# dlwns147/amq

Measured on AMD Instinct MI355X. Metric: decode tokens/s, Llama-2-7B AMQ mixed 2/3/4-bit avg-3-bit, batch 1, higher is better.
Workload: dtype f16; 1 GPU; Llama-2-7B shapes, synthesized avg-3.0-bit per-layer arch (bits_usage 2.982), batch 1 decode after a 64-token prefill, one stream per GPU; parallelism=replicas x1, prompt=64, group_size=128

## Files before the change

amq_amd/csrc/amq_decode.hip:

```cpp
#include <type_traits>
#include "amq_common.cuh"
#include "amq_kernels.h"

namespace amq {

__device__ __forceinline__ float wave_sum_f(float v) {
#pragma unroll
    for (int off = 32; off > 0; off >>= 1) v += __shfl_xor(v, off);
    return v;
}
__device__ __forceinline__ float wave_max_f(float v) {
#pragma unroll
    for (int off = 32; off > 0; off >>= 1) v = fmaxf(v, __shfl_xor(v, off));
    return v;
}

template <bool FRAG>
__global__ __launch_bounds__(256) void rmsnorm_kernel(const _Float16* x, const _Float16* gamma, _Float16* y, int M, int K, float eps) {
    __shared__ float red[4];
    const int m = blockIdx.x;
    const bool live = m < M;
    const _Float16* xr = x + (size_t)(live ? m : 0) * K;
    float ss = 0.f;
    for (int c = threadIdx.x; c < (K >> 3); c += 256) {
// ... 75 lines not shown
                *(h8*)(xlm + 8 * c) = r;
            }
        }
    }
    __syncthreads();
    const int gw = blockIdx.x * WV + wave, nw = gridDim.x * WV;
    const int steps = (K + 511) >> 9;
    for (int row = gw; row < N; row += nw) {
        const _Float16* wr = W + (size_t)row * K + 8 * lane;
        float acc[M];
#pragma unroll
        for (int m = 0; m < M; ++m) acc[m] = 0.f;
        for (int s = 0; s < steps; s += 4) {
            u4 buf[4];
#pragma unroll
            for (int j = 0; j < 4; ++j)
                if (s + j < steps && (s + j) * 512 + 8 * lane < K) buf[j] = AMQ_STREAM_LOAD((const u4*)(wr + (size_t)(s + j) * 512));
#pragma unroll
            for (int j = 0; j < 4; ++j) {
                if (s + j < steps && (s + j) * 512 + 8 * lane < K) {
                    const uint32_t wv[4] = {buf[j].x, buf[j].y, buf[j].z, buf[j].w};
#pragma unroll
                    for (int m = 0; m < M; ++m) {
                        const h8 xv = *(const h8*)(xl + (size_t)m * K + (s + j) * 512 + 8 * lane);
#pragma unroll
                        for (int p = 0; p < 4; ++p) {
                            h2 xp = {xv[2 * p], xv[2 * p + 1]};
                            acc[m] = __builtin_amdgcn_fdot2(as_h2(wv[p]), xp, acc[m], false);
                        }
                    }
                }
            }
        }
#pragma unroll
        for (int m = 0; m < M; ++m) {
            const float t = wave_sum_f(acc[m]);
            if (lane == 0) {
                _Float16 o = (_Float16)t;
                if (bias) o = o + bias[row];
                y[(size_t)m * N + row] = o;
            }
        }
    }
}

template <bool NORM, int M>
static hipError_t launch_gemv_f16w_m(const void* x, const void* W, const void* bias, void* y, const void* gamma, float eps,
                                     int N, int K, hipStream_t st) {
    const size_t lds = (size_t)M * K * 2 + 64;
    constexpr int WV = M == 1 ? F16W_WAVES : 16;
    auto k = gemv_f16w_kernel<NORM, M, WV>;
    if (lds > 64 * 1024) {
        hipError_t e = hipFuncSetAttribute((const void*)k, hipFuncAttributeMaxDynamicSharedMemorySize, (int)lds);
        if (e != hipSuccess) return e;
    }
    hipLaunchKernelGGL(k, dim3(M == 1 ? 1024 : 512), dim3(WV * 64), lds, st, (const _Float16*)x, (const _Float16*)W, (const _Float16*)bias,
                       (_Float16*)y, (const _Float16*)gamma, eps, N, K);
    return hipGetLastError();
}

template <bool NORM>
static hipError_t launch_gemv_f16w_n(const void* x, const void* W, const void* bias, void* y, const void* gamma, float eps,
                                     int M, int N, int K, hipStream_t st) {
    switch (M) {
        case 1: return launch_gemv_f16w_m<NORM, 1>(x, W, bias, y, gamma, eps, N, K, st);
        case 2: return launch_gemv_f16w_m<NORM, 2>(x, W, bias, y, gamma, eps, N, K, st);
        case 3: return launch_gemv_f16w_m<NORM, 3>(x, W, bias, y, gamma, eps, N, K, st);
        case 4: return launch_gemv_f16w_m<NORM, 4>(x, W, bias, y, gamma, eps, N, K, st);
        case 5: return launch_gemv_f16w_m<NORM, 5>(x, W, bias, y, gamma, eps, N, K, st);
        case 6: return launch_gemv_f16w_m<NORM, 6>(x, W, bias, y, gamma, eps, N, K, st);
        case 7: return launch_gemv_f16w_m<NORM, 7>(x, W, bias, y, gamma, eps, N, K, st);
        default: return launch_gemv_f16w_m<NORM, 8>(x, W, bias, y, gamma, eps, N, K, st);
    }
}

hipError_t launch_gemv_f16w(const void* x, const void* W, const void* bias, void* y, const void* gamma, float eps,
                            int N, int K, hipStream_t st, int M) {
    StreamDevice sd_(st);
    if (gamma) return launch_gemv_f16w_n<true>(x, W, bias, y, gamma, eps, M, N, K, st);
    return launch_gemv_f16w_n<false>(x, W, bias, y, nullptr, eps, M, N, K, st);
}

constexpr int TAIL_MAX_SUPPRESS = 8;
template <bool SEQ>
__global__ __launch_bounds__(1024) void decode_tail_kernel(const _Float16* logits, int vocab, const _Float16* embed, int hidden,
                                                            long long* token, int* pos, _Float16* x, const _Float16* rope_table,
                                                            _Float16* rope_cur, int rope_rows, const int* suppress) {
    __shared__ float smax[16];
    __shared__ int sidx[16];
    __shared__ int stok, spos;
    const int tid = threadIdx.x;
    logits += (size_t)blockIdx.x * vocab;
    token += blockIdx.x;
    x += (size_t)blockIdx.x * hidden;
    if (SEQ) {
        pos = (int*)((char*)pos + (size_t)blockIdx.x * STEP_STRIDE);
        if (rope_cur) rope_cur = (_Float16*)((char*)rope_cur + (size_t)blockIdx.x * STEP_STRIDE);
    } else if (blockIdx.x != 0) rope_cur = nullptr;
    float best = -INFINITY;
    int bi = 0x7fffffff;
    int sup[TAIL_MAX_SUPPRESS];
#pragma unroll
    for (int j = 0; j < TAIL_MAX_SUPPRESS; ++j) sup[j] = suppress ? suppress[j] : -1;
    auto allowed = [&](int idx) {
        bool ok = true;
#pragma unroll
        for (int j = 0; j < TAIL_MAX_SUPPRESS; ++j) ok = ok && idx != sup[j];
        return ok;
    };
    const int chunks = vocab >> 3;
    for (int c = tid; c < chunks; c += 1024) {
        const h8 v = *(const h8*)(logits + 8 * c);
#pragma unroll
        for (int e = 0; e < 8; ++e) {
            const float f = (float)v[e];
            if (f > best && (!suppress || allowed(8 * c + e))) { best = f; bi = 8 * c + e; }
        }
    }
    for (int i = 8 * chunks + tid; i < vocab; i += 1024) {
        const float f = (float)logits[i];
        if ((f > best || (f == best && i < bi)) && (!suppress || allowed(i))) { best = f; bi = i; }
    }
#pragma unroll
    for (int off = 32; off > 0; off >>= 1) {
        const float ob = __shfl_xor(best, off);
        const int oi = __shfl_xor(bi, off);
        if (ob > best || (ob == best && oi < bi)) { best = ob; bi = oi; }
    }
    if ((tid & 63) == 0) { smax[tid >> 6] = best; sidx[tid >> 6] = bi; }
    __syncthreads();
    if (tid == 0) {
        float b = smax[0];
        int ix = sidx[0];
        for (int w = 1; w < 16; ++w)
            if (smax[w] > b || (smax[w] == b && sidx[w] < ix)) { b = smax[w]; ix = sidx[w]; }
        if (ix == 0x7fffffff) ix = 0;
        stok = ix;
        token[0] = (long long)ix;
        if (SEQ || blockIdx.x == 0) {
            spos = pos[0] + 1;
            if (rope_table && spos > rope_rows) spos = rope_rows;
            pos[0] = spos;
        }
    }
    __syncthreads();
    if (rope_cur && tid < 128) {
        const int rr = spos < rope_rows ? spos : rope_rows - 1;
        rope_cur[tid] = rope_table[(size_t)rr * 128 + tid];
    }
    const _Float16* row = embed + (size_t)stok * hidden;
    for (int c = tid; c < (hidden >> 3); c += 1024) *(h8*)(x + 8 * c) = *(const h8*)(row + 8 * c);
}

hipError_t launch_decode_tail(const void* logits, int vocab, const void* embed, int hidden, void* token, void* pos, void* x,
                              const void* rope_table, void* rope_cur, int rope_rows, hipStream_t st, int batch, const void* suppress, bool seq) {
    hipLaunchKernelGGL(seq ? decode_tail_kernel<true> : decode_tail_kernel<false>, dim3(batch), dim3(1024), 0, st, (const _Float16*)logits, vocab,
                       (const _Float16*)embed, hidden, (long long*)token, (int*)pos, (_Float16*)x, (const _Float16*)rope_table, (_Float16*)rope_cur,
                       rope_rows, (const int*)suppress);
    return hipGetLastError();
}

template <bool SEQ>
__global__ __launch_bounds__(256) void set_token_kernel(const long long* token_in, int n_in, const _Float16* embed, int vocab, int hidden, long long* token,
                                                         const int* pos, _Float16* x, const _Float16* rope_table, _Float16* rope_cur, int rope_rows) {
    const int b = blockIdx.x, tid = threadIdx.x;
    long long t = token_in[n_in == 1 ? 0 : b];
    t = t < 0 ? 0 : t >= vocab ? vocab - 1 : t;
    if (tid == 0) token[b] = t;
    if (SEQ) {
        pos = (const int*)((const char*)pos + (size_t)b * STEP_STRIDE);
        if (rope_cur) rope_cur = (_Float16*)((char*)rope_cur + (size_t)b * STEP_STRIDE);
    }
    if ((SEQ || b == 0) && rope_cur && tid < 128) {
        int p = pos[0];
        p = p < 0 ? 0 : p < rope_rows ? p : rope_rows - 1;
        rope_cur[tid] = rope_table[(size_t)p * 128 + tid];
    }
    const _Float16* row = embed + (size_t)t * hidden;
    _Float16* xr = x + (size_t)b * hidden;
    for (int c = tid; c < (hidden >> 3); c += 256) *(h8*)(xr + 8 * c) = *(const h8*)(row + 8 * c);
}

hipError_t launch_set_token(const void* token_in, int n_in, const void* embed, int vocab, int hidden, void* token, const void* pos, void* x,
                            const void* rope_table, void* rope_cur, int rope_rows, int batch, hipStream_t st, bool seq) {
    hipLaunchKernelGGL(seq ? set_token_kernel<true> : set_token_kernel<false>, dim3(batch), dim3(256), 0, st, (const long long*)token_in, n_in,
                       (const _Float16*)embed, vocab, hidden, (long long*)token, (const int*)pos, (_Float16*)x, (const _Float16*)rope_table,
                       (_Float16*)rope_cur, rope_rows);
    return hipGetLastError();
}

constexpr int ATT_D = 128;

__device__ __forceinline__ void rope_cs(float theta, int pos, int i, _Float16* c16, _Float16* s16) {
    const float inv_freq = 1.0f / powf(theta, (float)(2 * i) / (float)ATT_D);
    float sn, cs;
    sincosf((float)pos * inv_freq, &sn, &cs);
    *c16 = (_Float16)cs;
    *s16 = (_Float16)sn;
}


constexpr int ATT_THREADS = 512;
constexpr int ATT_GROUPS = ATT_THREADS / 16;
constexpr int ATT_PF = 12;
#ifndef AMQ_ATT_SPEC
#define AMQ_ATT_SPEC 2
#endif
constexpr int ATT_SPEC = AMQ_ATT_SPEC;

struct AttnRest {
    void* out; const void* rope_table; int pos; float rope_theta;
#ifdef AMQ_STAMP
    unsigned long long* stamps;
#endif
};
struct AttnRestQkn : AttnRest { QkNorm nrm; };
template <bool QKN> using AttnRestT = std::conditional_t<QKN, AttnRestQkn, AttnRest>;
#ifdef AMQ_STAMP
extern unsigned long long* g_stamp_ptr;
#define ATT_STAMP(slot_) do { if (rest.stamps && threadIdx.x == 0) rest.stamps[(size_t)blockIdx.x * 16 + (slot_)] = __builtin_amdgcn_s_memrealtime(); } while (0)
#else
#define ATT_STAMP(slot_) do { } while (0)
#endif

constexpr int ATT_ROWS_MAX = 8;
constexpr int ATT_ROWS_LDS = 2 * (ATT_ROWS_MAX - 1) * ATT_D * 2;
template <bool SEQ, bool ROWS = false, bool QKN = false>
__global__ __launch_bounds__(ATT_THREADS) void attn_decode_kernel(void* p_kc, void* p_vc, const void* p_state, int p_heads,
                                                                   int p_max_seq, const void* p_q, const void* p_k,
                                                                   const void* p_v, AttnRestT<QKN> rest) {
    const void* const p_state0 = p_state;
    if (SEQ) p_state = (const char*)p_state + (size_t)blockIdx.y * STEP_STRIDE;
    extern __shared__ __attribute__((aligned(16))) unsigned char smem[];
    _Float16* qs = (_Float16*)smem;
    _Float16* ks = (_Float16*)smem + ATT_D;
    _Float16* vs = (_Float16*)smem + 2 * ATT_D;
    float* sc = (float*)(smem + 6 * ATT_D);
    __shared__ float red[2 * ATT_THREADS / 64];
    __shared__ float part[ATT_GROUPS][ATT_D];
// ... 137 lines not shown
        if (ATT_GROUPS * i < T) {
            const int t = grp + ATT_GROUPS * i;
            float sv;
            if constexpr (ROWS) {
                h8 kv = krow[i];
                if (t == pos) kv = knew;
                else if (t >= p0 && t < pos) kv = *(const h8*)(kd + (t - p0) * ATT_D + 8 * l16);
                sv = score(kv);
            } else sv = score(t == pos ? knew : krow[i]);
            if (t < T && l16 == 0) sc[t] = sv;
        }
    }
    for (int t = grp + ATT_GROUPS * ATT_PF; t < T; t += ATT_GROUPS) {
        h8 kv;
        if constexpr (ROWS) kv = (t == pos) ? knew : t >= p0 ? *(const h8*)(kd + (t - p0) * ATT_D + 8 * l16) : *(const h8*)(kc + (size_t)t * ATT_D + 8 * l16);
        else kv = (t == pos) ? knew : *(const h8*)(kc + (size_t)t * ATT_D + 8 * l16);
        const float sv = score(kv);
        if (l16 == 0) sc[t] = sv;
    }
    __syncthreads();
    ATT_STAMP(3);
    float lmax = -INFINITY;
    for (int t = tid; t < T; t += ATT_THREADS) lmax = fmaxf(lmax, sc[t]);
    lmax = wave_max_dpp(lmax);
    if ((tid & 63) == 0) red[tid >> 6] = lmax;
    __syncthreads();
    float gmax = red[0];
#pragma unroll
    for (int w = 1; w < ATT_THREADS / 64; ++w) gmax = fmaxf(gmax, red[w]);
    float lsum = 0.f;
    for (int t = tid; t < T; t += ATT_THREADS) {
        const float e = __expf(sc[t] - gmax);
        sc[t] = e;
        lsum += e;
    }
    lsum = wave_sum_dpp(lsum);
    if ((tid & 63) == 0) red[ATT_THREADS / 64 + (tid >> 6)] = lsum;
    __syncthreads();
    float tot = 0.f;
#pragma unroll
    for (int w = 0; w < ATT_THREADS / 64; ++w) tot += red[ATT_THREADS / 64 + w];
    const float inv = 1.0f / tot;
    ATT_STAMP(4);

    float o[8] = {0, 0, 0, 0, 0, 0, 0, 0};
    const h8 vnew = *(const h8*)(vs + 8 * l16);
#pragma unroll
    for (int i = 0; i < ATT_PF; ++i) {
        const int t = grp + ATT_GROUPS * i;
        if (ATT_GROUPS * i < T && t < T) {
            const _Float16 p16 = (_Float16)(sc[t] * inv);
            h8 vv;
            if constexpr (ROWS) {
                vv = vrow[i];
                if (t == pos) vv = vnew;
                else if (t >= p0 && t < pos) vv = *(const h8*)(vd + (t - p0) * ATT_D + 8 * l16);
            } else vv = (t == pos) ? vnew : vrow[i];
#pragma unroll
            for (int e = 0; e < 8; ++e) o[e] += (float)p16 * (float)vv[e];
        }
    }
    for (int t = grp + ATT_GROUPS * ATT_PF; t < T; t += ATT_GROUPS) {
        const _Float16 p16 = (_Float16)(sc[t] * inv);
        h8 vv;
        if constexpr (ROWS) vv = (t == pos) ? vnew : t >= p0 ? *(const h8*)(vd + (t - p0) * ATT_D + 8 * l16) : *(const h8*)(vc + (size_t)t * ATT_D + 8 * l16);
        else vv = (t == pos) ? vnew : *(const h8*)(vc + (size_t)t * ATT_D + 8 * l16);
#pragma unroll
        for (int e = 0; e < 8; ++e) o[e] += (float)p16 * (float)vv[e];
    }
#pragma unroll
    for (int e = 0; e < 8; ++e) part[grp][8 * l16 + e] = o[e];
    __syncthreads();
    ATT_STAMP(5);
    if (tid < ATT_D) {
        float acc = 0.f;
#pragma unroll
        for (int g = 0; g < ATT_GROUPS; ++g) acc += part[g][tid];
        _Float16* out = (_Float16*)rest.out + ((size_t)b * n_heads + h) * ATT_D;
        out[tid] = (_Float16)acc;
    }
    ATT_STAMP(6);
}

struct AttnSplit { float* ws; int* tickets; int n_splits; };
constexpr int ATT_WS_STRIDE = ATT_D + 4;

#ifndef AMQ_ATT_NT
#define AMQ_ATT_NT 1
#endif
#if AMQ_ATT_NT
#define ATT_KV_LOAD(p) __builtin_nontemporal_load((const h8*)(p))
#else
#define ATT_KV_LOAD(p) (*(const h8*)(p))
#endif
template <int RING, bool SEQ, bool ROWS = false, bool QKN = false>
__global__ __launch_bounds__(ATT_THREADS) void attn_decode_split_kernel(void* p_kc, void* p_vc, const void* p_state, int p_heads,
                                                                         int p_max_seq, const void* p_q, const void* p_k,
                                                                         const void* p_v, AttnRestT<QKN> rest, AttnSplit sp) {
    const void* const p_state0 = p_state;
    if (SEQ) p_state = (const char*)p_state + (size_t)blockIdx.y * STEP_STRIDE;
    extern __shared__ __attribute__((aligned(16))) unsigned char smem[];
    _Float16* qs = (_Float16*)smem;
    _Float16* ks = (_Float16*)smem + ATT_D;
    _Float16* vs = (_Float16*)smem + 2 * ATT_D;
    float* sc = (float*)(smem + 6 * ATT_D);
    __shared__ float red[2 * ATT_THREADS / 64];
    __shared__ float part[ATT_GROUPS][ATT_D];
    __shared__ int last_flag;
    const int b = blockIdx.y, z = blockIdx.z, tid = threadIdx.x;
    const int cb = ROWS ? 0 : b;
    const int n_heads = p_heads & 0xFF, n_kv_heads = (p_heads >> 8) & 0xFF, max_seq = p_max_seq;
    int h = blockIdx.x;
    if (n_kv_heads != n_heads && (n_kv_heads & 7) == 0) {
        const int G = n_heads / n_kv_heads, x = h & 7, j = h >> 3;
        h = (x + 8 * (j / G)) * G + j % G;
    }
    const bool cur_mode = (p_heads >> 16) & 1;
    const void* p_cur = cur_mode ? p_state : nullptr;
    int pos;
    if (cur_mode) pos = *(const int*)((const char*)p_state + 256);
    else if (p_state) pos = *(const int*)p_state;
    else pos = rest.pos;
    const int group = n_heads / n_kv_heads;
    const int kvh = h / group;
    const int grp = tid >> 4, l16 = tid & 15;
    const _Float16* q = (const _Float16*)p_q + ((size_t)b * n_heads + h) * ATT_D;
    const _Float16* kn = (const _Float16*)p_k + ((size_t)b * n_kv_heads + kvh) * ATT_D;
    const _Float16* vn = (const _Float16*)p_v + ((size_t)b * n_kv_heads + kvh) * ATT_D;
    _Float16* kc = (_Float16*)p_kc + ((size_t)cb * n_kv_heads + kvh) * (size_t)max_seq * ATT_D;
    _Float16* vc = (_Float16*)p_vc + ((size_t)cb * n_kv_heads + kvh) * (size_t)max_seq * ATT_D;

    _Float16 q0 = 0, q1 = 0, k0 = 0, k1 = 0, v0 = 0, v1 = 0;
    h2 cs_cur = {(_Float16)1.f, (_Float16)0.f}, cs_tab = {(_Float16)1.f, (_Float16)0.f};
    _Float16 gq0 = 0, gq1 = 0, gk0 = 0, gk1 = 0;
    if (tid < 64) {
        q0 = q[tid]; q1 = q[tid + 64];
        k0 = kn[tid]; k1 = kn[tid + 64];
        if (p_cur) cs_cur = ((const h2*)p_cur)[tid];
        v0 = vn[tid]; v1 = vn[tid + 64];
        if constexpr (QKN) {
            const _Float16* const gq = (const _Float16*)rest.nrm.q_gamma;
            const _Float16* const gk = (const _Float16*)rest.nrm.k_gamma;
            gq0 = gq[tid]; gq1 = gq[tid + 64];
            gk0 = gk[tid]; gk1 = gk[tid + 64];
        }
    }
    const int p0 = ROWS ? pos - b : pos;
    if (pos < 0 || pos >= max_seq || (ROWS && p0 < 0)) {
        if (cur_mode && tid == 0 && z == 0) *(int*)((char*)const_cast<void*>(p_state) + 260) = 1;
        return;
    }
    const int T = pos + 1;
    int chunk = (((T + sp.n_splits - 1) / sp.n_splits) + 31) & ~31;
    chunk = chunk < ATT_MIN_CHUNK ? ATT_MIN_CHUNK : chunk;
    const int n_act = (T + chunk - 1) / chunk;
    if (z >= n_act) return;
    const int t0 = z * chunk;
    const int t1 = t0 + chunk < T ? t0 + chunk : T;
    const int Tl = t1 - t0;
    const bool has_new = t1 == T;
    if (tid < 64 && !p_cur && rest.rope_table) cs_tab = ((const h2*)rest.rope_table)[(size_t)pos * 64 + tid];
    const int last_old = ROWS ? (p0 > 0 ? p0 - 1 : 0) : (pos > 0 ? pos - 1 : 0);
    int chunk_max = (((max_seq + sp.n_splits - 1) / sp.n_splits) + 31) & ~31;
    chunk_max = chunk_max < ATT_MIN_CHUNK ? ATT_MIN_CHUNK : chunk_max;
    _Float16* const kd = (_Float16*)(smem + 6 * ATT_D + (size_t)chunk_max * 4);
    _Float16* const vd = kd + (ATT_ROWS_MAX - 1) * ATT_D;
// ... 406 lines not shown
    for (int e = 0; e < 8; ++e) {
        const float gf = (float)gv[e];
        const _Float16 sg = (_Float16)(gf / (1.0f + __expf(-gf)));
        r[e] = sg * uv[e];
    }
    o[idx] = r;
}

hipError_t launch_silu_mul(const void* gate, const void* up, void* out, long n, hipStream_t st) {
    const long n8 = n >> 3;
    hipLaunchKernelGGL(silu_mul_kernel, dim3((unsigned)((n8 + 255) / 256)), dim3(256), 0, st, (const h8*)gate, (const h8*)up,
                       (h8*)out, n8);
    return hipGetLastError();
}

static int att_chunk_max(int max_seq, int n_splits) {
    int c = (((max_seq + n_splits - 1) / n_splits) + 31) & ~31;
    return c < ATT_MIN_CHUNK ? ATT_MIN_CHUNK : c;
}

template <bool QKN>
static AttnRestT<QKN> attn_rest(const AttnArgs& a, void* stamps) {
    AttnRestT<QKN> rest{};
    rest.out = a.out; rest.rope_table = a.rope_table; rest.pos = a.pos; rest.rope_theta = a.rope_theta;
#ifdef AMQ_STAMP
    rest.stamps = (unsigned long long*)stamps;
#endif
    (void)stamps;
    if constexpr (QKN) rest.nrm = a.norm;
    return rest;
}

template <int RING, bool QKN = false>
static hipError_t launch_attn_decode_split_ring(const AttnArgs& a, int batch, int n_splits, void* ws, void* tickets, size_t lds, hipStream_t st) {
    const auto kern = a.rows ? attn_decode_split_kernel<RING, true, true, QKN> : a.seq ? attn_decode_split_kernel<RING, true, false, QKN> : attn_decode_split_kernel<RING, false, false, QKN>;
    if (a.rows) lds += ATT_ROWS_LDS;
    if (lds > 64 * 1024) {
        hipError_t e = hipFuncSetAttribute((const void*)kern, hipFuncAttributeMaxDynamicSharedMemorySize, (int)lds);
        if (e != hipSuccess) return e;
    }
    const AttnRestT<QKN> rest = attn_rest<QKN>(a, nullptr);
    AttnSplit sp{(float*)ws, (int*)tickets, n_splits};
    const bool cur = a.rope_cur != nullptr;
    hipLaunchKernelGGL(kern, dim3(a.n_heads, batch, n_splits), dim3(ATT_THREADS), lds, st, a.kcache, a.vcache,
                       cur ? a.rope_cur : (const void*)a.pos_dev, a.n_heads | (a.n_kv_heads << 8) | ((int)cur << 16), a.max_seq,
                       a.q, a.k, a.v, rest, sp);
    return hipGetLastError();
}

hipError_t launch_attn_decode_split(const AttnArgs& a, int batch, int n_splits, void* ws, void* tickets, hipStream_t st) {
    if (!a.rows && attn_decode_takes_gqa(a.n_heads, a.n_kv_heads, a.max_seq, n_splits)) return launch_attn_decode_gqa(a, batch, n_splits, ws, tickets, st);
    StreamDevice sd_(st);
    const size_t lds = 6 * ATT_D + (size_t)att_chunk_max(a.max_seq, n_splits) * 4;
#ifndef AMQ_ATT_RING_WIDE
#define AMQ_ATT_RING_WIDE 12
#endif
#ifndef AMQ_ATT_RING_NARROW
#define AMQ_ATT_RING_NARROW 4
#endif
    const bool wide = (long)a.n_heads * batch * n_splits <= 256;
    if (a.norm.q_gamma) {
        if (wide) return launch_attn_decode_split_ring<AMQ_ATT_RING_WIDE, true>(a, batch, n_splits, ws, tickets, lds, st);
        return launch_attn_decode_split_ring<AMQ_ATT_RING_NARROW, true>(a, batch, n_splits, ws, tickets, lds, st);
    }
    if (wide) return launch_attn_decode_split_ring<AMQ_ATT_RING_WIDE>(a, batch, n_splits, ws, tickets, lds, st);
    return launch_attn_decode_split_ring<AMQ_ATT_RING_NARROW>(a, batch, n_splits, ws, tickets, lds, st);
}

template <bool QKN>
static hipError_t launch_attn_decode_t(const AttnArgs& a, int batch, hipStream_t st) {
    StreamDevice sd_(st);
    const size_t lds = a.rows ? ((6 * ATT_D + (size_t)a.max_seq * 4 + 15) & ~(size_t)15) + ATT_ROWS_LDS : 6 * ATT_D + (size_t)a.max_seq * 4;
    const auto kern = a.rows ? attn_decode_kernel<true, true, QKN> : a.seq ? attn_decode_kernel<true, false, QKN> : attn_decode_kernel<false, false, QKN>;
    if (lds > 64 * 1024) {
        hipError_t e = hipFuncSetAttribute((const void*)kern, hipFuncAttributeMaxDynamicSharedMemorySize, (int)lds);
        if (e != hipSuccess) return e;
    }
#ifdef AMQ_STAMP
    const AttnRestT<QKN> rest = attn_rest<QKN>(a, g_stamp_ptr);
#else
    const AttnRestT<QKN> rest = attn_rest<QKN>(a, nullptr);
#endif
    const bool cur = a.rope_cur != nullptr;
    hipLaunchKernelGGL(kern, dim3(a.n_heads, batch), dim3(ATT_THREADS), lds, st, a.kcache, a.vcache,
                       cur ? a.rope_cur : (const void*)a.pos_dev, a.n_heads | (a.n_kv_heads << 8) | ((int)cur << 16), a.max_seq,
                       a.q, a.k, a.v, rest);
    return hipGetLastError();
}

hipError_t launch_attn_decode(const AttnArgs& a, int batch, hipStream_t st) {
    return a.norm.q_gamma ? launch_attn_decode_t<true>(a, batch, st) : launch_attn_decode_t<false>(a, batch, st);
}

}
```

amq_amd/llama.py:

```python
import math
from typing import NamedTuple

import torch

from . import ops
from .arch import MODEL_CONFIGS, arch_bits, rope_inv_freq, uniform_arch
from .hqq_format import HQQWeights

EPS = 1e-5
ROPE_THETA = 10000.0


class _Lin:
    __slots__ = ("qn", "mn", "bits", "mode", "N", "K", "bias", "perm", "out_ids", "W_out", "Kp")

    def __init__(self, qn, mn, bits, mode, N, K, bias=None, perm=None, out_ids=None, W_out=None, Kp=None):
        self.qn, self.mn, self.bits, self.mode, self.N, self.K, self.bias = qn, mn, bits, mode, N, K, bias
        self.perm, self.out_ids, self.W_out, self.Kp = perm, out_ids, W_out, K if Kp is None else Kp

    @property
    def owq(self):
        return self.W_out is not None

    def seg(self, y, residual=None, act=False):
# ... 44 lines not shown
            g = torch.cuda.CUDAGraph()
            keep = torch.zeros(1, device=dev)
            with torch.cuda.graph(g, stream=side, capture_error_mode="thread_local"):
                keep += 1
        side.synchronize()
    _GRAPH_STATE_PRIMED.add(key)


def capture_graph(dev, fn, restore=None):
    side = torch.cuda.Stream(device=dev)
    side.wait_stream(torch.cuda.current_stream(dev))
    with torch.cuda.stream(side):
        fn()
        side.synchronize()
        if restore is not None:
            restore()
        g = torch.cuda.CUDAGraph()
        with _no_gc(), torch.cuda.graph(g, stream=side, capture_error_mode="thread_local"):
            fn()
    torch.cuda.current_stream(dev).wait_stream(side)
    return g


def _ints(values, n, lo, hi, message):
    each = [int(values)] * n if isinstance(values, int) else [int(v) for v in (values.reshape(-1).tolist() if isinstance(values, torch.Tensor) else values)]
    if len(each) != n or not all(lo <= v <= hi for v in each):
        raise ValueError(message.format(got=each))
    return each


NORM_FUSED, NORM_LAUNCH, NORM_FROM_SUMS = "fused", "launch", "sums"
DOWN_FUSED, DOWN_GEMV, DOWN_GEMV_SUMS, DOWN_GEMM = "silu_mul prologue", "silu_mul + gemv", "silu_mul + gemv leaving sums", "silu_mul + gemm"


class StepPlan(NamedTuple):
    first_norm: str
    norm: str
    down: str
    staged: bool = False

    @property
    def block_norm(self):
        return self.first_norm if self.norm == NORM_FROM_SUMS and self.down != DOWN_GEMV_SUMS else self.norm


def step_plan(R, H, I, fine, rows_h, rows_i, rows_i_phased, norm_sums=True, norm_fused_rows=4, down_fused_rows=1, rows_q=None):
    own = NORM_LAUNCH if R > norm_fused_rows else NORM_FUSED
    sums = norm_sums and 2 <= R <= 8 and not fine and 2048 <= H <= 8192 and I >= 2048 and R <= rows_h and (rows_q is None or R <= rows_q)
    if R <= min(rows_i, down_fused_rows):
        down = DOWN_FUSED
    elif R <= rows_i_phased:
        down = DOWN_GEMV_SUMS if sums else DOWN_GEMV
    else:
        down = DOWN_GEMM
    return StepPlan(own, NORM_FROM_SUMS if sums else own, down)


class _held_back:

    def __init__(self, runner, ids, hold):
        self.runner, self.ids, self.held = runner, tuple(ids), bool(hold)

    def __enter__(self):
        self.before = self.runner.suppressed
        if self.held:
            self.runner.set_suppressed(self.before + tuple(e for e in self.ids if e not in self.before))
        return self

    def release(self):
        if self.held:
            self.runner.set_suppressed(self.before)
            self.held = False

    def __exit__(self, *exc):
        self.runner.set_suppressed(self.before)
        return False


class QuantLlama:
    ENGINE_MAX_SEQ = 512
    DOWN_FUSED_ROWS = 1
    NORM_FUSED_ROWS = 4
    GATE_ACT = True
    NORM_SUMS = True
    FUSE_QKV_ATTN = False
    ROWS_GQA_FROM = 2048
    kv_bits = 16
    ENGINE_DEFAULT = False
    all_logits = False
    fine = False
    owq = False

    @classmethod
    def rows_attention_grouped(cls, n_heads, n_kv_heads, max_seq):
        if cls.ROWS_GQA_FROM is None or n_kv_heads < 1 or n_heads % n_kv_heads:
            return False
        return 2 <= n_heads // n_kv_heads <= 16 and max_seq >= cls.ROWS_GQA_FROM

    def __init__(self, config, arch_linear=None, device="cuda:0", max_seq=256, seed=0, synthetic=True,
                 hqq_layers=None, dense=None, batch=1, engine=None, prebuilt=None, group=128, rope=None, ragged=False, lookup=0, ngram_max=2,
                 lookup_sampling=False, kv_bits=16):
        if isinstance(config, str):
            config = MODEL_CONFIGS[config]
        if kv_bits not in (8, 16):
            raise ValueError(f"kv_bits must be 16 (fp16 cache) or 8 (int8 rows with a scale per row), got {kv_bits!r}")
        self.kv_bits = int(kv_bits)
        if self.kv_bits == 8:
            if ragged:
                raise ValueError("kv_bits=8: the 8-bit attention kernel keeps one position for the batch: not offered with ragged=True")
            if lookup:
                raise ValueError("kv_bits=8: a verify step runs 2 .. 8 rows of one sequence, the 8-bit attention kernel one: not offered with lookup=")
            if config.get("qk_norm"):
                raise ValueError("kv_bits=8: the 8-bit attention kernel has no per-head q / k norm: not offered for a qk_norm model")
            if engine:
                raise ValueError("kv_bits=8: the decode engine reads an fp16 cache")
            if self.FUSE_QKV_ATTN:
                raise ValueError("kv_bits=8: the fused q/k/v + attention launch reads an fp16 cache")
        if not 1 <= int(batch) <= 8:
            raise ValueError("batch must be 1..8")
        self.B = int(batch)
        self.ragged = bool(ragged)
        self.lookup = int(lookup or 0)
        self.lookup_sampling = bool(lookup_sampling)
        if self.lookup_sampling and not self.lookup:
            raise ValueError("lookup_sampling: sampled verify steps need a runner built with lookup=D (a plain runner samples after set_sampling)")
        if self.lookup:
            if not 1 <= self.lookup <= ops.LOOKUP_MAX_ROWS - 1:
                raise ValueError(f"lookup: 1..{ops.LOOKUP_MAX_ROWS - 1} drafts per step (the 2 .. 8-row launches), got {lookup}")
            if not 1 <= int(ngram_max) <= 4:
                raise ValueError(f"ngram_max must be 1..4, got {ngram_max}")
            if self.B != 1:
                raise ValueError("lookup: the rows of a step are the drafts of ONE sequence (batch 1); batches are not served")
            if self.ragged:
                raise ValueError("lookup: a ragged runner's step-state blocks are sequences, a lookup runner's are the rows of one sequence: not offered with ragged=True")
            if engine:
                raise ValueError("lookup: the decode engine runs one row per launch; a verify step runs 2 .. 8")
            if self.FUSE_QKV_ATTN:
                raise ValueError("lookup: the fused q/k/v + attention launch runs one row; a verify step runs 2 .. 8")
        self.ngram_max = int(ngram_max)
        self.R = self.lookup + 1 if self.lookup else self.B
        if self.ragged and engine:
            raise ValueError("the decode engine keeps one position (batch 1): not offered with ragged=True")
        if self.ragged and self.FUSE_QKV_ATTN:
            raise ValueError("the fused q/k/v + attention launch keeps one position (batch 1): not offered with ragged=True")
        self.cfg = config
        self.dev = torch.device(device)
        _prime_graph_state(self.dev)
        self.H = config["hidden_size"]
        self.I = config["intermediate_size"]
        self.nh, self.nkv = config["num_heads"], config["num_kv_heads"]
        if config["head_dim"] != 128:
            raise ValueError("head_dim must be 128")
        self.kvd = self.nkv * 128
        self.qd = self.nh * 128
        self.qk_norm = bool(config.get("qk_norm"))
        self.nb = config["n_block"]
        self.vocab = config["vocab_size"]
        self.max_seq = max_seq
        self.eps = float(config.get("rms_norm_eps", EPS))
        self.theta = float(config.get("rope_theta", ROPE_THETA))
        arch_linear = arch_linear or uniform_arch(config, 4)["linear"]
        self.arch_linear = arch_linear
        gen = torch.Generator(device=self.dev).manual_seed(seed)
        dev = self.dev

        def lin(block, name):
# ... 184 lines not shown
            if "RMSNorm" not in type(m).__name__ or w is None or tuple(w.shape) != (128,):
                raise ValueError(f"{where}.{name}: expected an RMSNorm over the 128 values of a head, got {type(m).__name__}"
                                 f"{'' if w is None else ' of width ' + 'x'.join(str(d) for d in w.shape)}")
            m_eps = getattr(m, "variance_epsilon", getattr(m, "eps", None))
            if m_eps is None or float(m_eps) != eps:
                raise ValueError(f"{where}.{name}: eps {m_eps} is not the model's rms_norm_eps {eps} (the runner keeps one eps)")

    @classmethod
    def from_hf(cls, model, max_seq=256, batch=1, engine=None, ragged=False, lookup=0, ngram_max=2, lookup_sampling=False, kv_bits=16):
        from .quant_linear import HIPOWQLinear, HIPQuantLinear
        cfg, rope = cls.check_hf(model, max_seq)
        layers = model.model.layers
        pre, arch_linear = {}, {name: [] for name in cfg["linear"]}
        dev = None
        f16 = lambda t: t.detach() if t.dtype is torch.float16 else t.detach().to(torch.float16)
        for b, layer in enumerate(layers):
            for name in cfg["linear"]:
                parent, attr = name.split(".")
                m = getattr(getattr(layer, parent), attr)
                if isinstance(m, HIPOWQLinear) and m.inner.qweight.is_cuda:
                    i = m.inner
                    if i.is_bf16:
                        raise ValueError(f"model.layers.{b}.{name}: a bfloat16 module -- the decode runner is fp16")
                    if m.perm.dtype is not torch.int32 or m.out_ids.dtype is not torch.int32 or m.W_out.dtype is not torch.float16 or \
                            tuple(m.W_out.shape) != (m.outfeatures, m.n_out) or m.perm.numel() != i.infeatures or m.out_ids.numel() != m.n_out:
                        raise ValueError(f"model.layers.{b}.{name}: the OWQ layer's perm / out_ids / W_out do not have the shapes of its packed layer")
                    dev = dev or i.qweight.device
                    pre[(b, name)] = _Lin(i.qweight, i.meta, i.bits, i.mode, m.outfeatures, m.infeatures, None if i.bias is None else f16(i.bias),
                                          perm=m.perm.contiguous(), out_ids=m.out_ids.contiguous(), W_out=m.W_out.contiguous(), Kp=i.infeatures)
                    arch_linear[name].append(i.bits)
                    continue
                if not isinstance(m, HIPQuantLinear) or not m.qweight.is_cuda:
                    raise ValueError(f"model.layers.{b}.{name}: expected a HIPQuantLinear on the GPU (run prepare_for_inference first)")
                if m.is_bf16:
                    raise ValueError(f"model.layers.{b}.{name}: a bfloat16 module -- the decode runner is fp16 (the reference's kernels are, ft.py:62); "
                                     "bf16 models run through the modules' own forward")
                dev = dev or m.qweight.device
                pre[(b, name)] = _Lin(m.qweight, m.meta, m.bits, m.mode, m.outfeatures, m.infeatures, None if m.bias is None else f16(m.bias))
                arch_linear[name].append(m.bits)
        dense = {"embed": f16(model.model.embed_tokens.weight), "lm_head": f16(model.lm_head.weight), "norm": f16(model.model.norm.weight),
                 "ln1": [f16(l.input_layernorm.weight) for l in layers], "ln2": [f16(l.post_attention_layernorm.weight) for l in layers]}
        if cfg.get("qk_norm"):
            dense["qn"] = [f16(l.self_attn.q_norm.weight).contiguous() for l in layers]
            dense["kn"] = [f16(l.self_attn.k_norm.weight).contiguous() for l in layers]
        return cls(cfg, arch_linear, device=dev, max_seq=max_seq, dense=dense, batch=batch, engine=engine, prebuilt=pre, synthetic=False, rope=rope,
                   ragged=ragged, lookup=lookup, ngram_max=ngram_max, lookup_sampling=lookup_sampling, kv_bits=kv_bits)

    def linear_bytes_per_token(self):
        return sum(blk[name].nbytes() for blk in self.blocks for name in self.cfg["linear"])

    def total_bytes_per_token(self, context):
        kv = 2 * self.nb * self.nkv * (ops.KV8_ROW_BYTES if self.kv_bits == 8 else 256) * context
        return self.linear_bytes_per_token() + self.lm_head.numel() * 2 + kv

    def _step(self, sampled=False):
        H, plan = self.H, self.plan
        if plan.staged:
            return self._step_staged(sampled)
        if self.engine is not None:
            self.engine.step()
            ops.gemv_f16w(self.x.reshape(-1), self.lm_head, gamma=self.norm, eps=self.eps, out=self.logits)
            self._tail(sampled)
            return
        if self.ragged and self.fuse_qkv_attn:
            raise ValueError("the fused q/k/v + attention launch keeps one position (batch 1): not offered with ragged=True")
        from_sums = plan.norm == NORM_FROM_SUMS
        first = plan.first_norm
        for blk in self.blocks:
            if self.fuse_qkv_attn:
                ops.gemv_qkv_attn(self.x, [blk["self_attn.q_proj"].seg(self.q.view(-1)), blk["self_attn.k_proj"].seg(self.k.view(-1)),
                                           blk["self_attn.v_proj"].seg(self.v.view(-1))], H, blk["ln1"], self.eps, blk["kc"], blk["vc"],
                                  self.att.view(-1), self.rope_cur, self.nh, self.nkv, self._tickets)
            else:
                self._behind_norm(first, blk["ln1"], [blk["self_attn.q_proj"].seg(self.q), blk["self_attn.k_proj"].seg(self.k),
                                                      blk["self_attn.v_proj"].seg(self.v)])
                if self.lookup:
                    ops.attn_decode_rows(self.q, self.k, self.v, blk["kc"], blk["vc"], self.att, self.rope_cur, self.pos, self.nh, self.nkv,
                                         grouped=self.rows_attention_grouped(self.nh, self.nkv, self.max_seq), **self._qkn(blk))
                elif self.kv_bits == 8:
                    ops.attn_decode_kv8(self.q, self.k, self.v, blk["kc8"], blk["ks"], blk["vc8"], blk["vs"], self.att, self.pos, self.nh, self.nkv,
                                        cur=self.rope_cur)
                else:
                    ops.attn_decode(self.q, self.k, self.v, blk["kc"], blk["vc"], self.att, self.pos, self.nh, self.nkv, self.theta,
                                    cur=self.rope_cur, **self._qkn(blk))
            o_proj, down = [blk["self_attn.o_proj"].seg(self.x, residual=self.x)], [blk["mlp.down_proj"].seg(self.x, residual=self.x)]
            if from_sums:
                ops.gemv_grouped_sums(self.att, o_proj, self.qd, sums_out=self.ss)
            else:
                ops.gemv_grouped(self.att, o_proj, self.qd)
            gate_act = self.GATE_ACT and self.R == 1 and plan.down == DOWN_FUSED and not self.fine
            self._behind_norm(plan.norm, blk["ln2"], [blk["mlp.gate_proj"].seg(self.gate, act=gate_act), blk["mlp.up_proj"].seg(self.up)])
            if plan.down == DOWN_FUSED:
                ops.gemv_grouped(self.gate, down, self.I, prologue=ops.PRO_SILU_MUL, x2=self.up, x_activated=gate_act)
            elif plan.down == DOWN_GEMV_SUMS:
                ops.gemv_grouped_sums(ops.silu_mul(self.gate, self.up, out=self.gate), down, self.I, sums_out=self.ss)
            elif plan.down == DOWN_GEMV:
                ops.gemv_grouped(ops.silu_mul(self.gate, self.up, out=self.gate), down, self.I)
            else:
                d = blk["mlp.down_proj"]
                ops.gemm(ops.silu_mul(self.gate, self.up, out=self.gate), d.qn, d.mn, d.bits, d.mode, d.N, d.K, bias=d.bias, residual=self.x, out=self.x)
            first = plan.block_norm
        ops.gemv_f16w(self.x.reshape(-1) if self.R == 1 else self.x, self.lm_head, gamma=self.norm, eps=self.eps, out=self.logits)
        self._tail(sampled)

    def _build_staged(self):
        R, dev = self.R, self.dev
        f16 = dict(dtype=torch.float16, device=dev)
        widths = {"self_attn.q_proj": self.H, "self_attn.k_proj": self.H, "self_attn.v_proj": self.H, "self_attn.o_proj": self.qd,
                  "mlp.gate_proj": self.H, "mlp.up_proj": self.H, "mlp.down_proj": self.I}
        self.xg = {n: torch.zeros(R * k, **f16) for n, k in widths.items()}
        self.act = torch.zeros(R, self.I, **f16)
        sets = []
        for blk in self.blocks:
            per = []
            for x, act, gamma, x2, plain_buf, names, outs, residual in (
                    (self.x, ops.OWQ_ACT_RMSNORM, blk["ln1"], None, self.xn, ("self_attn.q_proj", "self_attn.k_proj", "self_attn.v_proj"),
                     (self.q, self.k, self.v), None),
                    (self.att, ops.OWQ_ACT_NONE, None, None, self.att, ("self_attn.o_proj",), (self.x,), self.x),
                    (self.x, ops.OWQ_ACT_RMSNORM, blk["ln2"], None, self.xn, ("mlp.gate_proj", "mlp.up_proj"), (self.gate, self.up), None),
                    (self.gate, ops.OWQ_ACT_SILU_MUL, None, self.up, self.act, ("mlp.down_proj",), (self.x,), self.x)):
                K = x.shape[1]
                parts, gemvs, shared = [], [], False
                for n, y in zip(names, outs):
                    l = blk[n]
                    if l.owq:
                        xg = self.xg[n][:R * l.Kp].view(R, l.Kp)
                        parts.append(dict(perm=l.perm, out_ids=l.out_ids, W_out=l.W_out, xg=xg, y=y, residual=residual))
                        gemvs.append((l, xg, l.Kp, y, y))
                    else:
                        if not shared and plain_buf is not x:
                            parts.append(dict(xg=plain_buf))
                        shared = True
                        gemvs.append((l, plain_buf, K, y, residual))
                per.append((x, act, gamma, x2, ops.owq_stage_parts(parts, R, K) if parts else None, gemvs))
            sets.append(per)
        return sets

    def _step_staged(self, sampled):
        for blk, per in zip(self.blocks, self._staged):
            for i, (x, act, gamma, x2, arr, gemvs) in enumerate(per):
                if arr is not None:
                    ops.owq_stage_launch(x, self.R, x.shape[1], act, gamma, self.eps, x2, arr)
                for l, xin, K, y, residual in gemvs:
                    if self.R <= ops.gemv_max_rows(K, plain=True, norm=False):
                        ops.gemv_grouped(xin, [l.seg(y, residual=residual)], K)
                    else:
                        ops.gemm(xin, l.qn, l.mn, l.bits, l.mode, l.N, K, bias=l.bias, residual=residual, out=y)
                if i == 0:
                    if self.lookup:
                        ops.attn_decode_rows(self.q, self.k, self.v, blk["kc"], blk["vc"], self.att, self.rope_cur, self.pos, self.nh, self.nkv,
                                             grouped=self.rows_attention_grouped(self.nh, self.nkv, self.max_seq), **self._qkn(blk))
                    elif self.kv_bits == 8:
                        ops.attn_decode_kv8(self.q, self.k, self.v, blk["kc8"], blk["ks"], blk["vc8"], blk["vs"], self.att, self.pos, self.nh, self.nkv,
                                            cur=self.rope_cur)
                    else:
                        ops.attn_decode(self.q, self.k, self.v, blk["kc"], blk["vc"], self.att, self.pos, self.nh, self.nkv, self.theta,
                                        cur=self.rope_cur, **self._qkn(blk))
        ops.gemv_f16w(self.x.reshape(-1) if self.R == 1 else self.x, self.lm_head, gamma=self.norm, eps=self.eps, out=self.logits)
        self._tail(sampled)

    def _behind_norm(self, how, gamma, segments):
        if how == NORM_FROM_SUMS:
            ops.gemv_grouped_sums(self.x, segments, self.H, gamma=gamma, eps=self.eps, sums_in=self.ss)
        elif how == NORM_LAUNCH:
            ops.gemv_grouped(ops.rmsnorm(self.x, gamma, self.eps, out=self.xn), segments, self.H)
        else:
            ops.gemv_grouped(self.x, segments, self.H, prologue=ops.PRO_RMSNORM, gamma=gamma, eps=self.eps)

    def _tail(self, sampled):
        if self.lookup and sampled:
            if not self.lookup_sampling:
                raise ValueError("lookup: speculative decoding here is greedy (the sampled tail draws one token per row)")
            ops.decode_tail_lookup_sample(self.logits, self.embed, self.token, self.pos, self.x, self.lookup_state, self.history, self.rope_tab,
                                          self.rope_cur, self.sample_state, suppress=self.suppress)
        elif self.lookup:
            ops.decode_tail_lookup(self.logits, self.embed, self.token, self.pos, self.x, self.lookup_state, self.history, self.rope_tab, self.rope_cur,
                                   suppress=self.suppress)
        elif sampled:
            ops.decode_tail_sample(self.logits, self.embed, self.token, self.pos, self.x, self.sample_state, table=self.rope_tab, cur=self.rope_cur,
                                   suppress=self.suppress)
        else:
            ops.decode_tail(self.logits, self.embed, self.token, self.pos, self.x, table=self.rope_tab, cur=self.rope_cur, suppress=self.suppress)

    EOS_POLL_STEPS = 16

    def _write_sampling_state(self):
        if self.sample_state is None:
            self.sample_state = ops.new_sampling_state(self.dev)
        if self.sampling is not None:
            ops.set_sampling_state(self.sample_state, eos_ids=self.eos, pad_id=self.pad_id, **self.sampling)
        else:
            ops.set_sampling_state(self.sample_state, top_k=1, eos_ids=self.eos, pad_id=self.pad_id, first_kept=True)

    def set_sampling(self, temperature=1.0, top_k=0, top_p=1.0, seed=0):
        if temperature is None:
            self.sampling = None
            return
        if self.lookup and not self.lookup_sampling:
            raise ValueError("lookup: speculative decoding here is greedy; sampled speculative decoding (rejection sampling) is not served")
        self.sampling = dict(temperature=float(temperature), top_k=int(top_k), top_p=float(top_p), seed=int(seed))
        self._write_sampling_state()

    def set_eos(self, ids=(), pad_id=0):
        ids = tuple(int(i) for i in ids)
        if len(ids) > 8:
            raise ValueError("at most 8 EOS ids")
        self.eos, self.pad_id = ids, int(pad_id)
        if self.sample_state is not None:
            self._write_sampling_state()

    def _sampled_tail(self):
        return self.sampling is not None or self._greedy_eos

    def _first_token(self):
        if self.lookup:
            return self._lookup_first_token(self._prompt_len, sampled=True)
        tok = ops.sample(self.logits, self.sample_state, suppress=self.suppress, flags=ops.SAMPLE_ADVANCE | ops.SAMPLE_EOS)
        self.set_token(tok)

    def unfinished(self):
        return int(self.sample_state[24].item())

    def set_suppressed(self, ids=()):
        ids = tuple(int(i) for i in ids)
        if len(ids) > 8:
            raise ValueError("at most 8 suppressed token ids")
        if ids == self.suppressed:
            return
        self.suppress.copy_(torch.tensor(ids + (-1,) * (8 - len(ids)), dtype=torch.int32))
        self.suppressed = ids

    def _argmax(self, logits):
        m = torch.zeros(self.vocab + 1, dtype=torch.float32, device=logits.device)
        m.index_fill_(0, torch.where(self.suppress >= 0, self.suppress, self.vocab).to(torch.int64), float("-inf"))
        return torch.argmax(logits.float() + m[:self.vocab], dim=-1)

    def set_pos(self, pos):
        if self.ragged and not isinstance(pos, int) and (not isinstance(pos, torch.Tensor) or pos.numel() > 1 or self.B == 1):
            each = _ints(pos, self.B, 0, self.max_seq, f"expected {self.B} positions inside the KV cache (max_seq={self.max_seq}), got {{got}}")
            self.pos.copy_(torch.tensor(each, dtype=torch.int32))
            self.host_pos = max(each)
            return
# ... 684 lines not shown
```

Measured before the change: 798.7 tokens/s.

## Add short-context attention decode kernel and move pos/rope update early in tail

```diff
diff --git a/amq_amd/csrc/amq_decode.hip b/amq_amd/csrc/amq_decode.hip
--- a/amq_amd/csrc/amq_decode.hip
+++ b/amq_amd/csrc/amq_decode.hip
@@ -181,7 +181,7 @@
 }
 
 constexpr int TAIL_MAX_SUPPRESS = 8;
-template <bool SEQ>
+template <bool SEQ, bool EARLY = false>
 __global__ __launch_bounds__(1024) void decode_tail_kernel(const _Float16* logits, int vocab, const _Float16* embed, int hidden,
                                                             long long* token, int* pos, _Float16* x, const _Float16* rope_table,
                                                             _Float16* rope_cur, int rope_rows, const int* suppress) {
@@ -196,6 +196,17 @@
         pos = (int*)((char*)pos + (size_t)blockIdx.x * STEP_STRIDE);
         if (rope_cur) rope_cur = (_Float16*)((char*)rope_cur + (size_t)blockIdx.x * STEP_STRIDE);
     } else if (blockIdx.x != 0) rope_cur = nullptr;
+    if constexpr (EARLY) {
+        if (tid >= 1024 - 64 && (SEQ || blockIdx.x == 0)) {
+            int np = pos[0] + 1;
+            if (rope_table && np > rope_rows) np = rope_rows;
+            if (rope_cur) {
+                const int rr = np < rope_rows ? np : rope_rows - 1;
+                ((h2*)rope_cur)[tid - (1024 - 64)] = ((const h2*)rope_table)[(size_t)rr * 64 + (tid - (1024 - 64))];
+            }
+            if (tid == 1024 - 64) pos[0] = np;
+        }
+    }
     float best = -INFINITY;
     int bi = 0x7fffffff;
     int sup[TAIL_MAX_SUPPRESS];
@@ -236,14 +247,14 @@
         if (ix == 0x7fffffff) ix = 0;
         stok = ix;
         token[0] = (long long)ix;
-        if (SEQ || blockIdx.x == 0) {
+        if (!EARLY && (SEQ || blockIdx.x == 0)) {
             spos = pos[0] + 1;
             if (rope_table && spos > rope_rows) spos = rope_rows;
             pos[0] = spos;
         }
     }
     __syncthreads();
-    if (rope_cur && tid < 128) {
+    if (!EARLY && rope_cur && tid < 128) {
         const int rr = spos < rope_rows ? spos : rope_rows - 1;
         rope_cur[tid] = rope_table[(size_t)rr * 128 + tid];
     }
@@ -253,7 +264,8 @@
 
 hipError_t launch_decode_tail(const void* logits, int vocab, const void* embed, int hidden, void* token, void* pos, void* x,
                               const void* rope_table, void* rope_cur, int rope_rows, hipStream_t st, int batch, const void* suppress, bool seq) {
-    hipLaunchKernelGGL(seq ? decode_tail_kernel<true> : decode_tail_kernel<false>, dim3(batch), dim3(1024), 0, st, (const _Float16*)logits, vocab,
+    const auto kern = seq ? decode_tail_kernel<true> : decode_tail_kernel<false, true>;
+    hipLaunchKernelGGL(kern, dim3(batch), dim3(1024), 0, st, (const _Float16*)logits, vocab,
                        (const _Float16*)embed, hidden, (long long*)token, (int*)pos, (_Float16*)x, (const _Float16*)rope_table, (_Float16*)rope_cur,
                        rope_rows, (const int*)suppress);
     return hipGetLastError();
@@ -557,6 +569,162 @@
     ATT_STAMP(6);
 }
 
+__global__ __launch_bounds__(ATT_THREADS) void attn_decode_short_kernel(void* p_kc, void* p_vc, const void* p_state, int p_heads,
+                                                                         int p_max_seq, const void* p_q, const void* p_k,
+                                                                         const void* p_v, AttnRest rest) {
+    extern __shared__ __attribute__((aligned(16))) unsigned char smem[];
+    float* sc = (float*)smem;
+    __shared__ float red[2 * ATT_THREADS / 64];
+    __shared__ float part[ATT_GROUPS][ATT_D];
+    const int h = blockIdx.x, b = blockIdx.y, tid = threadIdx.x;
+    const int n_heads = p_heads & 0xFF, n_kv_heads = (p_heads >> 8) & 0xFF, max_seq = p_max_seq;
+    const int pos_in = *(const int*)((const char*)p_state + 256);
+    const int group = n_heads / n_kv_heads;
+    const int kvh = h / group;
+    const int grp = tid >> 4, l16 = tid & 15;
+    const _Float16* q = (const _Float16*)p_q + ((size_t)b * n_heads + h) * ATT_D;
+    const _Float16* kn = (const _Float16*)p_k + ((size_t)b * n_kv_heads + kvh) * ATT_D;
+    const _Float16* vn = (const _Float16*)p_v + ((size_t)b * n_kv_heads + kvh) * ATT_D;
+    _Float16* kc = (_Float16*)p_kc + ((size_t)b * n_kv_heads + kvh) * (size_t)max_seq * ATT_D;
+    _Float16* vc = (_Float16*)p_vc + ((size_t)b * n_kv_heads + kvh) * (size_t)max_seq * ATT_D;
+
+    ATT_STAMP(0);
+    const h8 qa = *(const h8*)(q + 8 * l16), qb = *(const h8*)(q + 8 * (l16 ^ 8));
+    const h8 ka = *(const h8*)(kn + 8 * l16), kb = *(const h8*)(kn + 8 * (l16 ^ 8));
+    const h8 cs0 = ((const h8*)p_state)[2 * (l16 & 7)], cs1 = ((const h8*)p_state)[2 * (l16 & 7) + 1];
+    const h8 vnew = *(const h8*)(vn + 8 * l16);
+    h8 krow[ATT_PF], vrow[ATT_PF];
+#pragma unroll
+    for (int i = 0; i < ATT_SPEC; ++i) {
+        int t = grp + ATT_GROUPS * i;
+        t = t < max_seq - 1 ? t : max_seq - 1;
+        krow[i] = *(const h8*)(kc + (size_t)t * ATT_D + 8 * l16);
+    }
+    const bool pos_ok = pos_in >= 0 && pos_in < max_seq;
+    const int pos = pos_ok ? pos_in : 0;
+    const int T = pos + 1;
+    ATT_STAMP(1);
+    const int last_old = pos > 0 ? pos - 1 : 0;
+#pragma unroll
+    for (int i = ATT_SPEC; i < ATT_PF; ++i) {
+        if (ATT_GROUPS * i < pos) {
+            int t = grp + ATT_GROUPS * i;
+            t = t < last_old ? t : last_old;
+            krow[i] = *(const h8*)(kc + (size_t)t * ATT_D + 8 * l16);
+        }
+    }
+    auto load_v = [&](int i) {
+        if (ATT_GROUPS * i < pos) {
+            int t = grp + ATT_GROUPS * i;
+            t = t < last_old ? t : last_old;
+            vrow[i] = *(const h8*)(vc + (size_t)t * ATT_D + 8 * l16);
+        }
+    };
+    const bool low = l16 < 8;
+    h8 qv, knew;
+#pragma unroll
+    for (int e = 0; e < 8; ++e) {
+        const _Float16 c16 = e < 4 ? cs0[2 * e] : cs1[2 * e - 8], s16 = e < 4 ? cs0[2 * e + 1] : cs1[2 * e - 7];
+        const _Float16 qp = low ? -qb[e] : qb[e], kp = low ? -kb[e] : kb[e];
+        qv[e] = qa[e] * c16 + qp * s16;
+        knew[e] = ka[e] * c16 + kp * s16;
+    }
+    ATT_STAMP(2);
+
+    const float scale = rsqrtf((float)ATT_D);
+    auto dot8 = [&](const h8& kv) {
+        float s = 0.f;
+#pragma unroll
+        for (int e = 0; e < 4; ++e)
+            s = __builtin_amdgcn_fdot2((h2){qv[2 * e], qv[2 * e + 1]}, (h2){kv[2 * e], kv[2 * e + 1]}, s, false);
+        return s;
+    };
+    auto scaled = [&](float s) {
+        s = row16_sum(s);
+        return (float)(_Float16)((float)(_Float16)s * scale);
+    };
+    auto score = [&](const h8& kv) { return scaled(dot8(kv)); };
+    float dot[ATT_PF];
+#pragma unroll
+    for (int i = 0; i < ATT_PF; ++i)
+        if (ATT_GROUPS * i < T) dot[i] = dot8(grp + ATT_GROUPS * i == pos ? knew : krow[i]);
+#pragma unroll
+    for (int i = 0; i < ATT_PF; ++i) load_v(i);
+    float wmax = -INFINITY;
+#pragma unroll
+    for (int i = 0; i < ATT_PF; ++i) {
+        if (ATT_GROUPS * i < T) {
+            const int t = grp + ATT_GROUPS * i;
+            const float sv = scaled(dot[i]);
+            if (t < T && l16 == 0) { sc[t] = sv; wmax = fmaxf(wmax, sv); }
+        }
+    }
+    for (int t = grp + ATT_GROUPS * ATT_PF; t < T; t += ATT_GROUPS) {
+        const h8 kv = (t == pos) ? knew : *(const h8*)(kc + (size_t)t * ATT_D + 8 * l16);
+        const float sv = score(kv);
+        if (l16 == 0) { sc[t] = sv; wmax = fmaxf(wmax, sv); }
+    }
+    wmax = wave_max_dpp(wmax);
+    if ((tid & 63) == 0) red[tid >> 6] = wmax;
+    __syncthreads();
+    ATT_STAMP(3);
+    float gmax = red[0];
+#pragma unroll
+    for (int w = 1; w < ATT_THREADS / 64; ++w) gmax = fmaxf(gmax, red[w]);
+    float lsum = 0.f;
+    for (int t = tid; t < T; t += ATT_THREADS) {
+        const float e = __expf(sc[t] - gmax);
+        sc[t] = e;
+        lsum += e;
+    }
+    lsum = wave_sum_dpp(lsum);
+    if ((tid & 63) == 0) red[ATT_THREADS / 64 + (tid >> 6)] = lsum;
+    __syncthreads();
+    float tot = 0.f;
+#pragma unroll
+    for (int w = 0; w < ATT_THREADS / 64; ++w) tot += red[ATT_THREADS / 64 + w];
+    const float inv = 1.0f / tot;
+    ATT_STAMP(4);
+
+    float o[8] = {0, 0, 0, 0, 0, 0, 0, 0};
+#pragma unroll
+    for (int i = 0; i < ATT_PF; ++i) {
+        const int t = grp + ATT_GROUPS * i;
+        if (ATT_GROUPS * i < T && t < T) {
+            const _Float16 p16 = (_Float16)(sc[t] * inv);
+            const h8 vv = (t == pos) ? vnew : vrow[i];
+#pragma unroll
+            for (int e = 0; e < 8; ++e) o[e] += (float)p16 * (float)vv[e];
+        }
+    }
+    for (int t = grp + ATT_GROUPS * ATT_PF; t < T; t += ATT_GROUPS) {
+        const _Float16 p16 = (_Float16)(sc[t] * inv);
+        const h8 vv = (t == pos) ? vnew : *(const h8*)(vc + (size_t)t * ATT_D + 8 * l16);
+#pragma unroll
+        for (int e = 0; e < 8; ++e) o[e] += (float)p16 * (float)vv[e];
+    }
+#pragma unroll
+    for (int e = 0; e < 8; ++e) part[grp][8 * l16 + e] = o[e];
+    __syncthreads();
+    ATT_STAMP(5);
+    if (!pos_ok) {
+        if (tid == 0) *(int*)((char*)const_cast<void*>(p_state) + 260) = 1;
+        return;
+    }
+    if (h % group == 0 && grp == 0) {
+        *(h8*)(kc + (size_t)pos * ATT_D + 8 * l16) = knew;
+        *(h8*)(vc + (size_t)pos * ATT_D + 8 * l16) = vnew;
+    }
+    if (tid < ATT_D) {
+        float acc = 0.f;
+#pragma unroll
+        for (int g = 0; g < ATT_GROUPS; ++g) acc += part[g][tid];
+        _Float16* out = (_Float16*)rest.out + ((size_t)b * n_heads + h) * ATT_D;
+        out[tid] = (_Float16)acc;
+    }
+    ATT_STAMP(6);
+}
+
 struct AttnSplit { float* ws; int* tickets; int n_splits; };
 constexpr int ATT_WS_STRIDE = ATT_D + 4;
 
@@ -1129,6 +1297,18 @@
     const AttnRestT<QKN> rest = attn_rest<QKN>(a, nullptr);
 #endif
     const bool cur = a.rope_cur != nullptr;
+    if constexpr (!QKN) {
+        const auto al16 = [](const void* p) { return ((uintptr_t)p & 15) == 0; };
+        if (cur && !a.seq && !a.rows && al16(a.q) && al16(a.k) && al16(a.v) && al16(a.rope_cur)) {
+            if ((size_t)a.max_seq * 4 > 64 * 1024) {
+                hipError_t e = hipFuncSetAttribute((const void*)attn_decode_short_kernel, hipFuncAttributeMaxDynamicSharedMemorySize, a.max_seq * 4);
+                if (e != hipSuccess) return e;
+            }
+            hipLaunchKernelGGL(attn_decode_short_kernel, dim3(a.n_heads, batch), dim3(ATT_THREADS), (size_t)a.max_seq * 4, st, a.kcache, a.vcache,
+                               a.rope_cur, a.n_heads | (a.n_kv_heads << 8) | (1 << 16), a.max_seq, a.q, a.k, a.v, rest);
+            return hipGetLastError();
+        }
+    }
     hipLaunchKernelGGL(kern, dim3(a.n_heads, batch), dim3(ATT_THREADS), lds, st, a.kcache, a.vcache,
                        cur ? a.rope_cur : (const void*)a.pos_dev, a.n_heads | (a.n_kv_heads << 8) | ((int)cur << 16), a.max_seq,
                        a.q, a.k, a.v, rest);
diff --git a/amq_amd/llama.py b/amq_amd/llama.py
--- a/amq_amd/llama.py
+++ b/amq_amd/llama.py
@@ -150,6 +150,7 @@
     DOWN_FUSED_ROWS = 1
     NORM_FUSED_ROWS = 4
     GATE_ACT = True
+    ATTN_SHORT = True
     NORM_SUMS = True
     FUSE_QKV_ATTN = False
     ROWS_GQA_FROM = 2048
@@ -500,7 +501,7 @@
                                         cur=self.rope_cur)
                 else:
                     ops.attn_decode(self.q, self.k, self.v, blk["kc"], blk["vc"], self.att, self.pos, self.nh, self.nkv, self.theta,
-                                    cur=self.rope_cur, **self._qkn(blk))
+                                    **self._attn_where(), **self._qkn(blk))
             o_proj, down = [blk["self_attn.o_proj"].seg(self.x, residual=self.x)], [blk["mlp.down_proj"].seg(self.x, residual=self.x)]
             if from_sums:
                 ops.gemv_grouped_sums(self.att, o_proj, self.qd, sums_out=self.ss)
@@ -573,9 +574,14 @@
                                             cur=self.rope_cur)
                     else:
                         ops.attn_decode(self.q, self.k, self.v, blk["kc"], blk["vc"], self.att, self.pos, self.nh, self.nkv, self.theta,
-                                        cur=self.rope_cur, **self._qkn(blk))
+                                        **self._attn_where(), **self._qkn(blk))
         ops.gemv_f16w(self.x.reshape(-1) if self.R == 1 else self.x, self.lm_head, gamma=self.norm, eps=self.eps, out=self.logits)
         self._tail(sampled)
+
+    def _attn_where(self):
+        if self.ATTN_SHORT or self.rope_cur.dim() != 1:
+            return dict(cur=self.rope_cur)
+        return dict(table=self.rope_tab)
 
     def _behind_norm(self, how, gamma, segments):
         if how == NORM_FROM_SUMS:
```

New measurement: 798.2 tokens/s, median of 2. No clear change (-0.1%).
